# eglrp/fSGM

Measured on AMD Instinct MI355X. Metric: aggregated cost-volume voxel-paths/s (HxWxDx8 paths), KITTI 1242x375 D=128, higher is better.
Workload: dtype u8

## Files before the change

### fsgm_amd/csrc/epi_band.hip

```cpp
#include "epi_kernels.h"
#include "fsgm_device.h"
#include "epi_step.h"
#include <type_traits>
#include <stdlib.h>

namespace fsgm {

#ifndef FSGM_BAND_PF
#define FSGM_BAND_PF 2
#endif
#ifndef FSGM_BAND_PF2
#define FSGM_BAND_PF2 1
#endif
#ifndef FSGM_BAND_PF4
#define FSGM_BAND_PF4 3
#endif
#ifndef FSGM_BAND_PFE
#define FSGM_BAND_PFE 4
#endif
#ifndef FSGM_BAND_PFE2
#define FSGM_BAND_PFE2 2
#endif
#ifndef FSGM_BAND_R16
#define FSGM_BAND_R16 1
#endif
#ifndef FSGM_BAND_Y16
#define FSGM_BAND_Y16 0
#endif
#ifndef FSGM_BAND_RECLDS
#define FSGM_BAND_RECLDS 1
#endif
#ifndef FSGM_BAND_SLACK
#define FSGM_BAND_SLACK 32
#endif
#ifndef FSGM_BAND_WAVES
#define FSGM_BAND_WAVES 8
#endif
#ifndef FSGM_BAND_MINW
#define FSGM_BAND_MINW 4
#endif

__device__ __forceinline__ uint32_t pack_hi_bits(const uint32_t (&R)[8]) {
    constexpr uint32_t SEL_HI = 0x07030501u;
    const uint32_t h0 = __builtin_amdgcn_perm(R[1], R[0], SEL_HI), h1 = __builtin_amdgcn_perm(R[3], R[2], SEL_HI);
    const uint32_t h2 = __builtin_amdgcn_perm(R[5], R[4], SEL_HI), h3 = __builtin_amdgcn_perm(R[7], R[6], SEL_HI);
    return h0 | (h1 << 1) | (h2 << 2) | (h3 << 3);
}
__device__ __forceinline__ void unpack_p9(const uint4 v, const uint32_t bits, uint32_t (&R)[8]) {
    const uint32_t w[4] = {v.x, v.y, v.z, v.w};
#pragma unroll
    for (int k = 0; k < 4; k++) {
        const uint32_t hk = (bits >> k) & 0x01010101u;
        R[2 * k] = __builtin_amdgcn_perm(hk, w[k], 0x06020400u);
        R[2 * k + 1] = __builtin_amdgcn_perm(hk, w[k], 0x07030501u);
    }
}

template <int LPP, int NT>
__device__ __forceinline__ uint2 band_nb_entry(const uint32_t d) {
    constexpr uint32_t D = LPP * 16;
    const uint32_t lo = d > 0 ? srow_index<NT>(0, d - 1) * 2u : 0u, hi = d + 1 < D ? srow_index<NT>(0, d + 1) * 2u : 0u;
    return make_uint2(lo | (hi << 16), (d > 0 ? 0x0000FFFFu : 0u) | (d + 1 < D ? 0xFFFF0000u : 0u));
}
template <uint32_t X>
__device__ __forceinline__ uint32_t sconst() { uint32_t r; asm("s_mov_b32 %0, %1" : "=s"(r) : "i"(X)); return r; }

template <int LPP, int NT, bool STAGE>
__device__ __forceinline__ void band_wta_record(const uint32_t (&ST)[8], uint32_t* sRow, const uint2* sNb, int tid, int j,
                                                bool ok, uint8_t* recb, uint8_t* s0b, uint32_t pix,
                                                uint2* stg_rec, uint16_t* stg_s0) {
    srow_store<NT>(sRow, tid, ST);
    const uint32_t IDX[8] = {sconst<0x80000u>(), sconst<0x90001u>(), sconst<0xA0002u>(), sconst<0xB0003u>(),
                             sconst<0xC0004u>(), sconst<0xD0005u>(), sconst<0xE0006u>(), sconst<0xF0007u>()};
    uint32_t K[8];
#pragma unroll
    for (int i = 0; i < 8; i++) K[i] = (ST[i] << 4) | IDX[i];
    const uint32_t kmin = pk_min(pk_min3(K[0], K[1], K[2]), pk_min3(K[3], K[4], pk_min3(K[5], K[6], K[7])));
    const uint32_t k16 = min_halves(kmin);
    uint32_t key;
    asm("v_lshl_or_b32 %0, %1, 4, %2" : "=v"(key) : "v"(k16 & ~15u), "v"((k16 & 15u) | ((uint32_t)j << 4)));
    key = group_min_u32<LPP>(key);
    __builtin_amdgcn_wave_barrier();
    if (j == 0 && ok) {
        const uint2 nb = sNb[key & 0xFFu];
        const uint8_t* row = (const uint8_t*)sRow + tid * 16;
        u16x2 c;
        c[0] = *(const uint16_t*)(row + (nb.x & 0xFFFFu));
        c[1] = *(const uint16_t*)(row + (nb.x >> 16));
        const uint2 rec = make_uint2(__builtin_amdgcn_perm(0u, key, sconst<0x02010C00u>()),
                                     __builtin_bit_cast(uint32_t, c) & nb.y);
        if (STAGE) {
            *stg_rec = rec;
            *stg_s0 = (uint16_t)ST[0];
        } else {
            *(uint2*)(recb + pix * 8u) = rec;
            *(uint16_t*)(s0b + pix * 2u) = (uint16_t)ST[0];
        }
    }
}

template <int LPP, int MODE, int NWV, int PATHS, bool BITS, bool TAP, bool CHAIN>
__global__ __launch_bounds__(NWV * 64, FSGM_BAND_MINW) void band_kernel(BandArgs a) {
    constexpr bool UP = MODE != 0;
    constexpr bool P8 = PATHS == 8;
    constexpr int PXG = 64 / LPP;
    constexpr int R = NWV * PXG;
    constexpr int D = LPP * 16;
    constexpr int SKEW = P8 ? 2 : 1;
    constexpr int NST = P8 ? 3 : 1;
    constexpr int PF = P8 ? (MODE == 2 ? FSGM_BAND_PF2 : FSGM_BAND_PF) : FSGM_BAND_PF4;
    constexpr bool R16 = P8 && MODE == 0 && !CHAIN && FSGM_BAND_R16 != 0;
    constexpr int NSL = R16 ? 2 : NST;
    __shared__ uint2 sNb[MODE == 2 ? D : 1];
    __shared__ uint4 sR16[R16 ? 2 : 1][2][R16 ? (R + 1) * LPP : 1];
    __shared__ uint4 sSt[2][NSL][(R + 1) * LPP];
    __shared__ __attribute__((aligned(16))) uint32_t sRow[MODE == 2 ? NWV * 64 * 8 : 4];
    constexpr bool RECLDS = MODE == 2 && FSGM_BAND_RECLDS != 0 && LPP == 8;
    __shared__ uint2 sRec[RECLDS ? NWV * 64 : 1];
    __shared__ uint16_t sRs0[RECLDS ? NWV * 64 : 1];
    __shared__ uint32_t sTicket;

    const int tid = threadIdx.x, lane = tid & 63, wave = tid >> 6;
    const int g = lane / LPP, j = lane % LPP;
    const int r = wave * PXG + g;
    const int W = a.W, H = a.H, NP = W * H;
    int cband = 0;
    size_t f = blockIdx.x;
    if (CHAIN) {
        if (tid == 0) sTicket = atomicAdd(a.ticket, 1u);
        __syncthreads();
        const uint32_t t = __builtin_amdgcn_readfirstlane(sTicket);
        const uint32_t per = (uint32_t)a.group * (uint32_t)a.nbands, grp = t / per, rem = t - grp * per;
        const uint32_t fin = min((uint32_t)a.group, (uint32_t)a.frames - grp * (uint32_t)a.group);
        cband = (int)(rem / fin);
        f = (size_t)grp * a.group + rem % fin;
        if (cband >= a.nbands || f >= (size_t)a.frames) return;
    }
    const uint8_t* __restrict__ Cf = a.C + f * a.c_frame_stride;
    uint8_t* __restrict__ Yf = a.Y + f * a.y_frame_stride;
    constexpr bool Y16 = BITS && FSGM_BAND_Y16 != 0;
    uint8_t* __restrict__ Bf = BITS ? (uint8_t*)(a.Yb + f * a.yb_frame_stride) : nullptr;
    uint8_t* __restrict__ Ef = (uint8_t*)(a.edge + f * a.edge_frame_stride);
    const uint32_t tag = CHAIN ? a.tag : 0u;
    uint8_t* __restrict__ recb = MODE == 2 ? (uint8_t*)(a.rec + f * (size_t)NP) : nullptr;
    uint8_t* __restrict__ s0b = MODE == 2 ? (uint8_t*)(a.s0 + f * (size_t)NP) : nullptr;
    const uint32_t P1pk = (uint32_t)a.P1 * 0x10001u, P2 = (uint32_t)a.P2, P2pk = P2 * 0x10001u;
    const uint32_t Bpk = (P2 + (uint32_t)a.P1) * 0x10001u;
    const uint4 startP = make_uint4(P2 * 0x01010101u, P2 * 0x01010101u, P2 * 0x01010101u, P2 * 0x01010101u);
    const LaneSel sel = lane_sel<LPP>(j);
    const int elane = min(lane, NST * LPP - 1);

    if (MODE == 2 && tid < D) sNb[tid] = band_nb_entry<LPP, NWV * 64>((uint32_t)tid);

    auto pix_of = [&](int x, int y) -> int { const int p = y * W + x; return UP ? NP - 1 - p : p; };

    for (int yb = CHAIN ? cband * R : 0; yb < (CHAIN ? cband * R + 1 : H); yb += R) {
        const int Rp = min(R, H - yb);
        const int y = yb + r, yc = min(y, H - 1);
        const bool row_ok = r < Rp;
        const int nsteps = W + SKEW * (Rp - 1);
        const bool have_above = yb > 0, last_band = yb + R >= H;
        const bool loader = wave == 0 && lane < NST * LPP && have_above;
        const int r_lo = wave * PXG, r_hi = r_lo + PXG - 1;
        const int act_lo = SKEW * r_lo - (P8 ? 1 : 0), act_hi = W - 1 + SKEW * r_hi;
        const bool wave_rows = r_lo < Rp;
        const int pl_lo = SKEW * r_hi + 1, pl_hi = W - 2 + SKEW * r_lo;
        const bool wave_plain_rows = r_hi < Rp && yb + r_lo >= 1;

        auto vox_off = [&](int u) -> uint32_t {
            const int x = min(max(u - SKEW * r, 0), W - 1);
            return (uint32_t)pix_of(x, yc) * D + (uint32_t)j * 16;
        };
        auto bit_off = [&](int u) -> uint32_t {
            const int x = min(max(u - SKEW * r, 0), W - 1);
            return ((uint32_t)pix_of(x, yc) * LPP + (uint32_t)j) * 4u;
        };
        const uint32_t emap = (uint32_t)W * (NST * LPP) * 16u;
        const uint8_t* __restrict__ Ein = CHAIN ? Ef + (uint32_t)max(cband - 1, 0) * emap : Ef;
        uint8_t* __restrict__ Eout = CHAIN ? Ef + (uint32_t)cband * emap : Ef;
        auto edge_at = [&](int x) -> const uint8_t* { return Ein + ((uint32_t)min(max(x, 0), W - 1) * (NST * LPP) + (uint32_t)elane) * 16u; };
        bool gave_up = false;
        auto put_above = [&](const int par, const uint4 v) {
            if (R16 && elane / LPP == 2) {
                uint32_t S[8];
                unpack_p(v, S);
                sR16[par][0][elane % LPP] = make_uint4(S[0], S[1], S[2], S[3]);
                sR16[par][1][elane % LPP] = make_uint4(S[4], S[5], S[6], S[7]);
            } else {
                sSt[par][elane / LPP][elane % LPP] = v;
            }
        };
        auto fresh = [&](const uint4 v) -> bool { return (((v.x ^ tag) | (v.y ^ tag) | (v.z ^ tag) | (v.w ^ tag)) & 0x80808080u) == 0u; };
        auto eload = [&](const uint8_t* q) -> uint4 { return CHAIN ? edge_load((const uint4*)q) : load_nt(q); };
        auto settle = [&](uint4 v, const uint8_t* q, const bool mine) -> uint4 {
            if (CHAIN) {
                for (uint32_t spins = 0; !gave_up && !__all(!mine || fresh(v)); spins++) {
                    __builtin_amdgcn_s_sleep(8);
                    if (mine) v = edge_load((const uint4*)q);
                    if (spins > (1u << 18) || ((spins & 1023u) == 1023u && __hip_atomic_load(a.err, __ATOMIC_RELAXED, __HIP_MEMORY_SCOPE_AGENT) != 0u)) {
                        if (lane == 0) atomicOr(a.err, 1u);
                        gave_up = true;
                    }
                }
                v.x &= 0x7F7F7F7Fu; v.y &= 0x7F7F7F7Fu; v.z &= 0x7F7F7F7Fu; v.w &= 0x7F7F7F7Fu;
            }
            return v;
        };

        uint32_t FS[8];
#pragma unroll
        for (int i = 0; i < 8; i++) FS[i] = P2pk;
        uint4 hU = startP, hD1 = startP, hD2 = startP;
        if (P8 && have_above && wave == 0) {
            const bool mine = r == 0;
            const uint8_t* q0 = Ein + (uint32_t)(0 * LPP + j) * 16u;
            const uint8_t* q1 = Ein + (uint32_t)(1 * LPP + j) * 16u;
            const uint4 v0 = settle(mine ? eload(q0) : startP, q0, mine), v1 = settle(mine ? eload(q1) : startP, q1, mine);
            if (mine) { hU = v0; hD1 = v1; }
        }
        if (CHAIN && wave == 0 && have_above) {
            const uint8_t* q = edge_at(min(SKEW + FSGM_BAND_SLACK, W - 1));
            (void)settle(loader ? eload(q) : startP, q, loader);
        }
        if (wave == 0 && have_above) {
            const uint8_t* q = edge_at(SKEW - 1);
            const uint4 v = settle(loader ? eload(q) : startP, q, loader);
            if (loader) put_above(1, v);
        }
        uint4 ringC[PF], ringY[MODE == 2 ? PF : 1];
        constexpr int PFE = CHAIN ? (MODE == 2 ? FSGM_BAND_PFE2 : FSGM_BAND_PFE) : 1;
        uint4 ringE[PFE];
#pragma unroll
        for (int i = 0; i < PFE; i++) ringE[i] = startP;
        uint32_t ringB[MODE == 2 && BITS && !Y16 ? PF : 1];
        uint4 ringB4[MODE == 2 && Y16 ? PF : 1];
#pragma unroll
        for (int i = 0; i < PF; i++) {
            const uint32_t off = vox_off(i);
            ringC[i] = *(const uint4*)(Cf + off);
            if (MODE == 2) {
                ringY[i] = vol_load(Yf + off);
                if (Y16) ringB4[i] = vol_load(Bf + off);
                else if (BITS) ringB[i] = *(const uint32_t*)(Bf + bit_off(i));
            }
        }
        if (loader) {
#pragma unroll
            for (int i = 0; i < PFE; i++) ringE[i] = eload(edge_at(SKEW + i));
        }
        if constexpr (RECLDS) sRec[wave * 64 + lane] = make_uint2(0xFFFFFFFFu, 0xFFFFFFFFu);
        __syncthreads();

        auto do_step = [&](const int u, const uint4 cw, const uint4 cy, const uint32_t cb, const uint4 cb4, auto edge_tag) {
            constexpr bool EDGE = decltype(edge_tag)::value;
            const int par = u & 1;
            const int x = u - SKEW * r;
            const bool inside = !EDGE || (row_ok && x >= 0 && x < W);
            const int xc = EDGE ? min(max(x, 0), W - 1) : x;
            uint4 nNow, nLo, nHi;
            if constexpr (R16) { nLo = sR16[par ^ 1][0][r * LPP + j]; nHi = sR16[par ^ 1][1][r * LPP + j]; }
            else nNow = sSt[par ^ 1][P8 ? 2 : 0][r * LPP + j];
            uint32_t CP[8], Y[8], YS[8], S[8];
            unpack_cb(cw, CP, Bpk);
            const bool top = EDGE && y == 0;
            {
                const bool st = EDGE && x <= 0;
                if (st) {
#pragma unroll
                    for (int i = 0; i < 8; i++) FS[i] = P2pk;
                }
                step_b<LPP, EDGE>(FS, CP, YS, P1pk, P2, sel, st ? 0u : 0xFFFFu);
            }
            if (MODE == 2) {
                uint32_t E2[8];
                if (Y16) { E2[0] = cy.x; E2[1] = cy.y; E2[2] = cy.z; E2[3] = cy.w; E2[4] = cb4.x; E2[5] = cb4.y; E2[6] = cb4.z; E2[7] = cb4.w; }
                else if (BITS) unpack_p9(cy, cb, E2);
                else unpack_p(cy, E2);
#pragma unroll
                for (int i = 0; i < 8; i++) YS[i] += E2[i];
            }
            __builtin_amdgcn_sched_barrier(0);
            uint4 newU, newD, newR;
            {
                unpack_p(P8 ? hU : nNow, S);
                if (top) {
#pragma unroll
                    for (int i = 0; i < 8; i++) S[i] = P2pk;
                }
                step_b<LPP, EDGE>(S, CP, Y, P1pk, P2, sel, top ? 0u : 0xFFFFu);
                newU = pack_p(S);
                sSt[par][0][(r + 1) * LPP + j] = newU;
#pragma unroll
                for (int i = 0; i < 8; i++) YS[i] += Y[i];
            }
            __builtin_amdgcn_sched_barrier(0);
            if constexpr (P8) {
                {
                    const bool st = top || (EDGE && x <= 0);
                    unpack_p(hD2, S);
                    if (st) {
#pragma unroll
                        for (int i = 0; i < 8; i++) S[i] = P2pk;
                    }
                    step_b<LPP, EDGE>(S, CP, Y, P1pk, P2, sel, st ? 0u : 0xFFFFu);
                    newD = pack_p(S);
                    sSt[par][1][(r + 1) * LPP + j] = newD;
#pragma unroll
                    for (int i = 0; i < 8; i++) YS[i] += Y[i];
                    hD2 = hD1;
                    hD1 = sSt[par ^ 1][1][r * LPP + j];
                    hU = sSt[par ^ 1][0][r * LPP + j];
                }
                __builtin_amdgcn_sched_barrier(0);
                {
                    const bool st = top || (EDGE && x >= W - 1);
                    if (R16) { S[0] = nLo.x; S[1] = nLo.y; S[2] = nLo.z; S[3] = nLo.w; S[4] = nHi.x; S[5] = nHi.y; S[6] = nHi.z; S[7] = nHi.w; }
                    else unpack_p(nNow, S);
                    if (st) {
#pragma unroll
                        for (int i = 0; i < 8; i++) S[i] = P2pk;
                    }
                    step_b<LPP, EDGE>(S, CP, Y, P1pk, P2, sel, st ? 0u : 0xFFFFu);
                    if constexpr (R16) {
                        sR16[par][0][(r + 1) * LPP + j] = make_uint4(S[0], S[1], S[2], S[3]);
                        sR16[par][1][(r + 1) * LPP + j] = make_uint4(S[4], S[5], S[6], S[7]);
                        if (!last_band && r == R - 1) newR = pack_p(S);
                    } else {
                        newR = pack_p(S);
                        sSt[par][2][(r + 1) * LPP + j] = newR;
                    }
#pragma unroll
                    for (int i = 0; i < 8; i++) YS[i] += Y[i];
                }
            }
            if (!last_band && r == R - 1 && inside) {
                uint8_t* o = Eout + ((uint32_t)xc * (NST * LPP) + (uint32_t)j) * 16u;
                if (CHAIN) {
                    edge_store((uint4*)o, make_uint4(newU.x | tag, newU.y | tag, newU.z | tag, newU.w | tag));
                    if constexpr (P8) {
                        edge_store((uint4*)(o + LPP * 16), make_uint4(newD.x | tag, newD.y | tag, newD.z | tag, newD.w | tag));
                        edge_store((uint4*)(o + 2 * LPP * 16), make_uint4(newR.x | tag, newR.y | tag, newR.z | tag, newR.w | tag));
                    }
                } else {
                    *(uint4*)o = newU;
                    if constexpr (P8) { *(uint4*)(o + LPP * 16) = newD; *(uint4*)(o + 2 * LPP * 16) = newR; }
                }
            }
            if (MODE != 2) {
                if (inside) {
                    const uint32_t px = (uint32_t)pix_of(xc, yc);
                    if (Y16) {
                        vol_store(Yf + px * D + (uint32_t)j * 16, make_uint4(YS[0], YS[1], YS[2], YS[3]));
                        vol_store(Bf + px * D + (uint32_t)j * 16, make_uint4(YS[4], YS[5], YS[6], YS[7]));
                    } else {
                        vol_store(Yf + px * D + (uint32_t)j * 16, pack_p(YS));
                        if (BITS) *(uint32_t*)(Bf + (px * LPP + (uint32_t)j) * 4u) = pack_hi_bits(YS);
                    }
                }
            } else {
                uint32_t ST[8];
#pragma unroll
                for (int i = 0; i < 8; i++) ST[i] = CP[i] * (uint32_t)PATHS - YS[i];
                if constexpr (RECLDS)
                    band_wta_record<LPP, NWV * 64, true>(ST, sRow, sNb, tid, j, inside, recb, s0b, 0u, &sRec[wave * 64 + g * 8 + (u & 7)], &sRs0[wave * 64 + g * 8 + (u & 7)]);
                else
                    band_wta_record<LPP, NWV * 64, false>(ST, sRow, sNb, tid, j, inside, recb, s0b, (uint32_t)pix_of(xc, yc), nullptr, nullptr);
                if (TAP && inside) {
                    uint32_t* o = a.Sdbg + (f * (size_t)NP + pix_of(xc, yc)) * D + j * 16;
#pragma unroll
                    for (int i = 0; i < 8; i++) { o[i] = ST[i] & 0xFFFFu; o[i + 8] = ST[i] >> 16; }
                }
            }
        };
        auto flush_records = [&](const int u) {
            if constexpr (RECLDS) {
                __builtin_amdgcn_wave_barrier();
                const int fr = lane >> 3, fs = lane & 7;
                const uint2 rc = sRec[wave * 64 + lane];
                const uint16_t s0v = sRs0[wave * 64 + lane];
                sRec[wave * 64 + lane] = make_uint2(0xFFFFFFFFu, 0xFFFFFFFFu);
                const int uu = (u & ~7) + fs, rr = wave * PXG + fr;
                const int xx = uu - SKEW * rr;
                if (rc.x != 0xFFFFFFFFu) {
                    const uint32_t px = (uint32_t)pix_of(xx, yb + rr);
                    *(uint2*)(recb + px * 8u) = rc;
                    *(uint16_t*)(s0b + px * 2u) = s0v;
                }
                __builtin_amdgcn_wave_barrier();
            }
        };
        auto step = [&](const int u, const uint4 cw, const uint4 cy, const uint32_t cb, const uint4 cb4) {
            if (wave == 0 && have_above) {
                const uint4 v = settle(ringE[0], edge_at(u + SKEW), loader);
#pragma unroll
                for (int i = 0; i + 1 < PFE; i++) ringE[i] = ringE[i + 1];
                if (loader) {
                    put_above(u & 1, v);
                    ringE[PFE - 1] = eload(edge_at(u + PFE + SKEW));
                }
            }
            if (wave_rows && u >= act_lo && u <= act_hi) {
                if (wave_plain_rows && u >= pl_lo && u <= pl_hi) do_step(u, cw, cy, cb, cb4, std::false_type{});
                else do_step(u, cw, cy, cb, cb4, std::true_type{});
            }
            if constexpr (RECLDS) {
                if ((u & 7) == 7) flush_records(u);
            }
#ifndef FSGM_BAND_NOBAR
            __syncthreads();
#endif
        };

        int u0 = 0;
        for (; u0 + PF <= nsteps; u0 += PF) {
#pragma unroll
            for (int i = 0; i < PF; i++) {
                const int u = u0 + i;
                const uint4 cw = ringC[i];
                const uint4 cy = ringY[MODE == 2 ? i : 0];
                const uint32_t cb = ringB[MODE == 2 && BITS && !Y16 ? i : 0];
                const uint4 cb4 = ringB4[MODE == 2 && Y16 ? i : 0];
                const uint32_t off = vox_off(u + PF);
                ringC[i] = *(const uint4*)(Cf + off);
                if (MODE == 2) {
                    ringY[i] = vol_load(Yf + off);
                    if (Y16) ringB4[i] = vol_load(Bf + off);
                    else if (BITS) ringB[i] = *(const uint32_t*)(Bf + bit_off(u + PF));
                }
                step(u, cw, cy, cb, cb4);
            }
        }
#pragma unroll
        for (int i = 0; i < PF - 1; i++)
            if (u0 + i < nsteps) step(u0 + i, ringC[i], ringY[MODE == 2 ? i : 0], ringB[MODE == 2 && BITS && !Y16 ? i : 0], ringB4[MODE == 2 && Y16 ? i : 0]);
        if constexpr (RECLDS) {
            if ((nsteps & 7) != 0) flush_records(nsteps - 1);
        }
        if (!CHAIN) {
            asm volatile("s_waitcnt vmcnt(0)" ::: "memory");
            __syncthreads();
        }
    }
}

size_t band_edge_uint4s(int W, int D, int paths) { const int lpp = agg_packed_lpp(D); return (size_t)W * (paths == 8 ? 3 : 1) * lpp; }
size_t band_bits_u32s(int W, int H, int D) { return (size_t)W * H * agg_packed_lpp(D) * (FSGM_BAND_Y16 ? 4 : 1); }
bool band_needs_bits(int paths, int P1, int P2) { return paths == 8 && 4 * (P1 + P2) > 255; }
bool band_ok(int D, int paths, int P1, int P2, int cmax) {
    return agg_packed_lpp(D) != 0 && P1 >= 0 && P2 >= 0 && P1 + P2 <= 127 && (paths == 8 || paths == 4) && 16 * paths * (cmax + P2 + P1) + 15 < 0x7C00;
}

template <int LPP, int MODE>
static void launch_band_t(hipStream_t st, const BandArgs& a, int frames, int paths) {
    constexpr int NWV = FSGM_BAND_WAVES;
    const bool bits = band_needs_bits(paths, a.P1, a.P2);
    dim3 grid((unsigned)(a.chain ? frames * a.nbands : frames)), block(NWV * 64);
    if (MODE == 2 && a.Sdbg) {
        if (paths == 4)  hipLaunchKernelGGL((band_kernel<LPP, MODE, NWV, 4, false, MODE == 2, false>), grid, block, 0, st, a);
        else if (!bits)  hipLaunchKernelGGL((band_kernel<LPP, MODE, NWV, 8, false, MODE == 2, false>), grid, block, 0, st, a);
        else             hipLaunchKernelGGL((band_kernel<LPP, MODE, NWV, 8, true, MODE == 2, false>), grid, block, 0, st, a);
        return;
    }
    if (a.chain) {
        if (paths == 4)  hipLaunchKernelGGL((band_kernel<LPP, MODE, NWV, 4, false, false, true>), grid, block, 0, st, a);
        else if (!bits)  hipLaunchKernelGGL((band_kernel<LPP, MODE, NWV, 8, false, false, true>), grid, block, 0, st, a);
        else             hipLaunchKernelGGL((band_kernel<LPP, MODE, NWV, 8, true, false, true>), grid, block, 0, st, a);
        return;
    }
    if (paths == 4)  hipLaunchKernelGGL((band_kernel<LPP, MODE, NWV, 4, false, false, false>), grid, block, 0, st, a);
    else if (!bits)  hipLaunchKernelGGL((band_kernel<LPP, MODE, NWV, 8, false, false, false>), grid, block, 0, st, a);
    else             hipLaunchKernelGGL((band_kernel<LPP, MODE, NWV, 8, true, false, false>), grid, block, 0, st, a);
}

int band_rows(int D) { const int lpp = agg_packed_lpp(D); return lpp ? FSGM_BAND_WAVES * (64 / lpp) : 0; }

void launch_band(hipStream_t st, const BandArgs& a, int frames, int paths, int mode) {
#define FSGM_BAND(L) do { if (mode == 0) launch_band_t<L, 0>(st, a, frames, paths); else launch_band_t<L, 2>(st, a, frames, paths); } while (0)
    switch (agg_packed_lpp(a.D)) {
        case 1: FSGM_BAND(1); break;
        case 2: FSGM_BAND(2); break;
        case 4: FSGM_BAND(4); break;
        case 8: FSGM_BAND(8); break;
        case 16: FSGM_BAND(16); break;
        default: break;
    }
#undef FSGM_BAND
}

}
```

Before: 5940 billion.

## Use complemented-cost step with v_xad and ping-pong diagonal state in band SGM

Replaces the step_b recurrence with a new step_x that works on complemented costs: the cost is unpacked with plain byte perms and the add/subtract is folded into a single v_xad_u32 with a 0x7F constant, and the final cost sum is rebuilt with a shift plus a bias constant instead of a multiply-subtract. The diagonal history hD1/hD2 shift becomes a two-entry ping-pong indexed by step parity. To keep that parity static, the prefetch ring gets an extra slot in MODE 2 and the loop is unrolled to an even length. The aim is fewer VALU ops per voxel step and fewer register moves, at the cost of more registers for the larger ring and unroll, and a risk of subtle arithmetic mistakes in the complemented form (for example the tail loop reusing the same ring indexing).

```diff
diff --git a/fsgm_amd/csrc/epi_band.hip b/fsgm_amd/csrc/epi_band.hip
--- a/fsgm_amd/csrc/epi_band.hip
+++ b/fsgm_amd/csrc/epi_band.hip
@@ -53,6 +53,39 @@
         const uint32_t hk = (bits >> k) & 0x01010101u;
         R[2 * k] = __builtin_amdgcn_perm(hk, w[k], 0x06020400u);
         R[2 * k + 1] = __builtin_amdgcn_perm(hk, w[k], 0x07030501u);
+    }
+}
+
+__device__ __forceinline__ void band_unpack_c(const uint4 w, uint32_t (&C)[8]) {
+    C[0] = __builtin_amdgcn_perm(w.z, w.x, 0x0C040C00u);
+    C[1] = __builtin_amdgcn_perm(w.z, w.x, 0x0C050C01u);
+    C[2] = __builtin_amdgcn_perm(w.z, w.x, 0x0C060C02u);
+    C[3] = __builtin_amdgcn_perm(w.z, w.x, 0x0C070C03u);
+    C[4] = __builtin_amdgcn_perm(w.w, w.y, 0x0C040C00u);
+    C[5] = __builtin_amdgcn_perm(w.w, w.y, 0x0C050C01u);
+    C[6] = __builtin_amdgcn_perm(w.w, w.y, 0x0C060C02u);
+    C[7] = __builtin_amdgcn_perm(w.w, w.y, 0x0C070C03u);
+}
+template <int LPP, bool MASKED, bool OUT_N>
+__device__ __forceinline__ void step_x(uint32_t (&S)[8], const uint32_t (&C)[8], uint32_t (&O)[8], const uint32_t P1pk,
+                                       const uint32_t P2pk, const uint32_t kx, const uint32_t K0, const LaneSel sel,
+                                       const bool start) {
+    uint32_t N[8], YB[8];
+    const uint32_t LT = __builtin_amdgcn_perm(S[7], (uint32_t)__builtin_amdgcn_mov_dpp((int)S[7], DPP_ROW_SHR1, 0xF, 0xF, true), sel.lo);
+    const uint32_t RT = __builtin_amdgcn_perm((uint32_t)__builtin_amdgcn_mov_dpp((int)S[0], DPP_ROW_SHL1, 0xF, 0xF, true), S[0], sel.hi);
+#pragma unroll
+    for (int i = 0; i < 8; i++) {
+        YB[i] = pk_max3(S[i] + P1pk, i ? S[i - 1] : LT, i < 7 ? S[i + 1] : RT);
+        asm("v_xad_u32 %0, %1, %2, %3" : "=v"(N[i]) : "v"(YB[i]), "s"(kx), "v"(C[i]));
+    }
+    const uint32_t mm = pk_min(pk_min3(N[0], N[1], N[2]), pk_min3(N[3], N[4], pk_min3(N[5], N[6], N[7])));
+    uint32_t mx = group_min_u32<LPP>(min_halves(mm));
+    if (MASKED && start) mx = K0;
+    const uint32_t p2m = __umul24(mx, 0x10001u) + P2pk;
+#pragma unroll
+    for (int i = 0; i < 8; i++) {
+        S[i] = pk_subs(p2m, N[i]);
+        O[i] = OUT_N ? N[i] : YB[i];
     }
 }
 
@@ -145,7 +178,8 @@
     uint8_t* __restrict__ recb = MODE == 2 ? (uint8_t*)(a.rec + f * (size_t)NP) : nullptr;
     uint8_t* __restrict__ s0b = MODE == 2 ? (uint8_t*)(a.s0 + f * (size_t)NP) : nullptr;
     const uint32_t P1pk = (uint32_t)a.P1 * 0x10001u, P2 = (uint32_t)a.P2, P2pk = P2 * 0x10001u;
-    const uint32_t Bpk = (P2 + (uint32_t)a.P1) * 0x10001u;
+    const uint32_t KX = sconst<0x007F007Fu>(), K0 = 127u - (P2 + (uint32_t)a.P1);
+    const uint32_t K1pk = (uint32_t)(PATHS * (a.P1 + a.P2) - (PATHS / 2) * 127) * 0x10001u;
     const uint4 startP = make_uint4(P2 * 0x01010101u, P2 * 0x01010101u, P2 * 0x01010101u, P2 * 0x01010101u);
     const LaneSel sel = lane_sel<LPP>(j);
     const int elane = min(lane, NST * LPP - 1);
@@ -210,13 +244,13 @@
         uint32_t FS[8];
 #pragma unroll
         for (int i = 0; i < 8; i++) FS[i] = P2pk;
-        uint4 hU = startP, hD1 = startP, hD2 = startP;
+        uint4 hU = startP, hDp[2] = {startP, startP};
         if (P8 && have_above && wave == 0) {
             const bool mine = r == 0;
             const uint8_t* q0 = Ein + (uint32_t)(0 * LPP + j) * 16u;
             const uint8_t* q1 = Ein + (uint32_t)(1 * LPP + j) * 16u;
             const uint4 v0 = settle(mine ? eload(q0) : startP, q0, mine), v1 = settle(mine ? eload(q1) : startP, q1, mine);
-            if (mine) { hU = v0; hD1 = v1; }
+            if (mine) { hU = v0; hDp[1] = v1; }
         }
         if (CHAIN && wave == 0 && have_above) {
             const uint8_t* q = edge_at(min(SKEW + FSGM_BAND_SLACK, W - 1));
@@ -227,13 +261,15 @@
             const uint4 v = settle(loader ? eload(q) : startP, q, loader);
             if (loader) put_above(1, v);
         }
-        uint4 ringC[PF], ringY[MODE == 2 ? PF : 1];
+        constexpr int NR = MODE == 2 && P8 ? PF + 1 : PF;
+        constexpr int UN = P8 && (NR & 1) ? 2 * NR : NR;
+        uint4 ringC[NR], ringY[MODE == 2 ? NR : 1];
         constexpr int PFE = CHAIN ? (MODE == 2 ? FSGM_BAND_PFE2 : FSGM_BAND_PFE) : 1;
         uint4 ringE[PFE];
 #pragma unroll
         for (int i = 0; i < PFE; i++) ringE[i] = startP;
-        uint32_t ringB[MODE == 2 && BITS && !Y16 ? PF : 1];
-        uint4 ringB4[MODE == 2 && Y16 ? PF : 1];
+        uint32_t ringB[MODE == 2 && BITS && !Y16 ? NR : 1];
+        uint4 ringB4[MODE == 2 && Y16 ? NR : 1];
 #pragma unroll
         for (int i = 0; i < PF; i++) {
             const uint32_t off = vox_off(i);
@@ -251,7 +287,7 @@
         if constexpr (RECLDS) sRec[wave * 64 + lane] = make_uint2(0xFFFFFFFFu, 0xFFFFFFFFu);
         __syncthreads();
 
-        auto do_step = [&](const int u, const uint4 cw, const uint4 cy, const uint32_t cb, const uint4 cb4, auto edge_tag) {
+        auto do_step = [&](const int u, const int hp, const uint4 cw, const uint4 cy, const uint32_t cb, const uint4 cb4, auto edge_tag) {
             constexpr bool EDGE = decltype(edge_tag)::value;
             const int par = u & 1;
             const int x = u - SKEW * r;
@@ -261,7 +297,7 @@
             if constexpr (R16) { nLo = sR16[par ^ 1][0][r * LPP + j]; nHi = sR16[par ^ 1][1][r * LPP + j]; }
             else nNow = sSt[par ^ 1][P8 ? 2 : 0][r * LPP + j];
             uint32_t CP[8], Y[8], YS[8], S[8];
-            unpack_cb(cw, CP, Bpk);
+            band_unpack_c(cw, CP);
             const bool top = EDGE && y == 0;
             {
                 const bool st = EDGE && x <= 0;
@@ -269,7 +305,7 @@
 #pragma unroll
                     for (int i = 0; i < 8; i++) FS[i] = P2pk;
                 }
-                step_b<LPP, EDGE>(FS, CP, YS, P1pk, P2, sel, st ? 0u : 0xFFFFu);
+                step_x<LPP, EDGE, MODE == 2>(FS, CP, YS, P1pk, P2pk, KX, K0, sel, st);
             }
             if (MODE == 2) {
                 uint32_t E2[8];
@@ -277,7 +313,7 @@
                 else if (BITS) unpack_p9(cy, cb, E2);
                 else unpack_p(cy, E2);
 #pragma unroll
-                for (int i = 0; i < 8; i++) YS[i] += E2[i];
+                for (int i = 0; i < 8; i++) YS[i] -= E2[i];
             }
             __builtin_amdgcn_sched_barrier(0);
             uint4 newU, newD, newR;
@@ -287,28 +323,27 @@
 #pragma unroll
                     for (int i = 0; i < 8; i++) S[i] = P2pk;
                 }
-                step_b<LPP, EDGE>(S, CP, Y, P1pk, P2, sel, top ? 0u : 0xFFFFu);
+                step_x<LPP, EDGE, MODE == 2>(S, CP, Y, P1pk, P2pk, KX, K0, sel, top);
                 newU = pack_p(S);
                 sSt[par][0][(r + 1) * LPP + j] = newU;
 #pragma unroll
-                for (int i = 0; i < 8; i++) YS[i] += Y[i];
+                for (int i = 0; i < 8; i++) YS[i] += MODE == 2 ? Y[i] + K1pk : Y[i];
             }
             __builtin_amdgcn_sched_barrier(0);
             if constexpr (P8) {
                 {
                     const bool st = top || (EDGE && x <= 0);
-                    unpack_p(hD2, S);
+                    unpack_p(hDp[hp], S);
                     if (st) {
 #pragma unroll
                         for (int i = 0; i < 8; i++) S[i] = P2pk;
                     }
-                    step_b<LPP, EDGE>(S, CP, Y, P1pk, P2, sel, st ? 0u : 0xFFFFu);
+                    step_x<LPP, EDGE, MODE == 2>(S, CP, Y, P1pk, P2pk, KX, K0, sel, st);
                     newD = pack_p(S);
                     sSt[par][1][(r + 1) * LPP + j] = newD;
 #pragma unroll
                     for (int i = 0; i < 8; i++) YS[i] += Y[i];
-                    hD2 = hD1;
-                    hD1 = sSt[par ^ 1][1][r * LPP + j];
+                    hDp[hp] = sSt[par ^ 1][1][r * LPP + j];
                     hU = sSt[par ^ 1][0][r * LPP + j];
                 }
                 __builtin_amdgcn_sched_barrier(0);
@@ -320,7 +355,7 @@
 #pragma unroll
                         for (int i = 0; i < 8; i++) S[i] = P2pk;
                     }
-                    step_b<LPP, EDGE>(S, CP, Y, P1pk, P2, sel, st ? 0u : 0xFFFFu);
+                    step_x<LPP, EDGE, MODE == 2>(S, CP, Y, P1pk, P2pk, KX, K0, sel, st);
                     if constexpr (R16) {
                         sR16[par][0][(r + 1) * LPP + j] = make_uint4(S[0], S[1], S[2], S[3]);
                         sR16[par][1][(r + 1) * LPP + j] = make_uint4(S[4], S[5], S[6], S[7]);
@@ -360,7 +395,7 @@
             } else {
                 uint32_t ST[8];
 #pragma unroll
-                for (int i = 0; i < 8; i++) ST[i] = CP[i] * (uint32_t)PATHS - YS[i];
+                for (int i = 0; i < 8; i++) ST[i] = (CP[i] << (P8 ? 2 : 1)) + YS[i];
                 if constexpr (RECLDS)
                     band_wta_record<LPP, NWV * 64, true>(ST, sRow, sNb, tid, j, inside, recb, s0b, 0u, &sRec[wave * 64 + g * 8 + (u & 7)], &sRs0[wave * 64 + g * 8 + (u & 7)]);
                 else
@@ -389,7 +424,7 @@
                 __builtin_amdgcn_wave_barrier();
             }
         };
-        auto step = [&](const int u, const uint4 cw, const uint4 cy, const uint32_t cb, const uint4 cb4) {
+        auto step = [&](const int u, const int hp, const uint4 cw, const uint4 cy, const uint32_t cb, const uint4 cb4) {
             if (wave == 0 && have_above) {
                 const uint4 v = settle(ringE[0], edge_at(u + SKEW), loader);
 #pragma unroll
@@ -400,8 +435,8 @@
                 }
             }
             if (wave_rows && u >= act_lo && u <= act_hi) {
-                if (wave_plain_rows && u >= pl_lo && u <= pl_hi) do_step(u, cw, cy, cb, cb4, std::false_type{});
-                else do_step(u, cw, cy, cb, cb4, std::true_type{});
+                if (wave_plain_rows && u >= pl_lo && u <= pl_hi) do_step(u, hp, cw, cy, cb, cb4, std::false_type{});
+                else do_step(u, hp, cw, cy, cb, cb4, std::true_type{});
             }
             if constexpr (RECLDS) {
                 if ((u & 7) == 7) flush_records(u);
@@ -411,28 +446,29 @@
 #endif
         };
 
+        auto ring_step = [&](const int u, const int i) {
+            const int k = i % NR, kl = (i + PF) % NR;
+            const uint4 cw = ringC[k];
+            const uint4 cy = ringY[MODE == 2 ? k : 0];
+            const uint32_t cb = ringB[MODE == 2 && BITS && !Y16 ? k : 0];
+            const uint4 cb4 = ringB4[MODE == 2 && Y16 ? k : 0];
+            const uint32_t off = vox_off(u + PF);
+            ringC[kl] = *(const uint4*)(Cf + off);
+            if (MODE == 2) {
+                ringY[kl] = vol_load(Yf + off);
+                if (Y16) ringB4[kl] = vol_load(Bf + off);
+                else if (BITS) ringB[kl] = *(const uint32_t*)(Bf + bit_off(u + PF));
+            }
+            step(u, i & 1, cw, cy, cb, cb4);
+        };
         int u0 = 0;
-        for (; u0 + PF <= nsteps; u0 += PF) {
-#pragma unroll
-            for (int i = 0; i < PF; i++) {
-                const int u = u0 + i;
-                const uint4 cw = ringC[i];
-                const uint4 cy = ringY[MODE == 2 ? i : 0];
-                const uint32_t cb = ringB[MODE == 2 && BITS && !Y16 ? i : 0];
-                const uint4 cb4 = ringB4[MODE == 2 && Y16 ? i : 0];
-                const uint32_t off = vox_off(u + PF);
-                ringC[i] = *(const uint4*)(Cf + off);
-                if (MODE == 2) {
-                    ringY[i] = vol_load(Yf + off);
-                    if (Y16) ringB4[i] = vol_load(Bf + off);
-                    else if (BITS) ringB[i] = *(const uint32_t*)(Bf + bit_off(u + PF));
-                }
-                step(u, cw, cy, cb, cb4);
-            }
-        }
-#pragma unroll
-        for (int i = 0; i < PF - 1; i++)
-            if (u0 + i < nsteps) step(u0 + i, ringC[i], ringY[MODE == 2 ? i : 0], ringB[MODE == 2 && BITS && !Y16 ? i : 0], ringB4[MODE == 2 && Y16 ? i : 0]);
+        for (; u0 + UN <= nsteps; u0 += UN) {
+#pragma unroll
+            for (int i = 0; i < UN; i++) ring_step(u0 + i, i);
+        }
+#pragma unroll
+        for (int i = 0; i < UN - 1; i++)
+            if (u0 + i < nsteps) ring_step(u0 + i, i);
         if constexpr (RECLDS) {
             if ((nsteps & 7) != 0) flush_records(nsteps - 1);
         }
```

Result: faster. 6086 billion, median of 6 (+2.4%).
